# ekzhu/datasketch

Hardware: AMD Instinct MI355X
Metric: MinHash signatures/sec (1M sets x 256 tokens, num_perm=128) (higher is better)
Workload: dtype u64

## Files before the change

### datasketch_amd/csrc/mhx_api.hip

```cpp
#include <algorithm>
#include <cmath>
#include <condition_variable>
#include <cstdlib>
#include <cstring>
#include <mutex>
#include <new>
#include <system_error>
#include <thread>
#include <vector>

#include "mhx_internal.h"

namespace mhx {

static thread_local std::string g_last_error;

void set_error(const char *fmt, ...) {
    char buf[1024];
    va_list ap;
    va_start(ap, fmt);
    vsnprintf(buf, sizeof(buf), fmt, ap);
    va_end(ap);
    g_last_error = buf;
}
// ... 263 lines not shown

int mhx_ctx::ensure_copy_streams() {
    if (!copy_in) MHX_HIP_CHECK(hipStreamCreateWithFlags(&copy_in, hipStreamNonBlocking));
    if (!copy_out) MHX_HIP_CHECK(hipStreamCreateWithFlags(&copy_out, hipStreamNonBlocking));
    return MHX_OK;
}

int mhx_ctx::ensure_redo(int64_t n_sets) {
    if (n_sets <= redo_capacity && d_redo) return MHX_OK;
    if (d_redo) {
        (void)hipStreamSynchronize(stream);
        (void)mhx::dev_free(d_redo);
        d_redo = nullptr;
        redo_capacity = 0;
    }
    const int64_t cap = std::max<int64_t>(n_sets + n_sets / 4, 1024);
    hipError_t e = mhx::dev_malloc(reinterpret_cast<void **>(&d_redo), (size_t)cap + 64);
    if (e != hipSuccess) {
        d_redo = nullptr;
        return fail(MHX_ERR_OOM, "redo flag allocation of %lld bytes failed: %s", (long long)cap, hipGetErrorString(e));
    }
    redo_capacity = cap;
    return MHX_OK;
}

int mhx_ctx::ensure_work() {
    if (d_work) return MHX_OK;
    hipError_t e = mhx::dev_malloc(reinterpret_cast<void **>(&d_work), mhx::kWorkBytes);
    if (e != hipSuccess) {
        d_work = nullptr;
        return fail(MHX_ERR_OOM, "work counter allocation failed: %s", hipGetErrorString(e));
    }
    MHX_HIP_CHECK(hipMemsetAsync(d_work, 0, mhx::kWorkBytes, stream));
    return MHX_OK;
}

extern "C" {

const char *mhx_last_error(void) { return mhx::g_last_error.c_str(); }

const char *mhx_version(void) { return "mhx 0.1.0 (gfx950)"; }

int mhx_device_count(int *count) {
    if (!count) return fail(MHX_ERR_INVALID, "count is NULL");
    int n = 0;
    hipError_t e = hipGetDeviceCount(&n);
    if (e != hipSuccess) {
        (void)hipGetLastError();
        *count = 0;
        return MHX_OK;
    }
    *count = n;
    return MHX_OK;
}

int mhx_ctx_create(int device, mhx_ctx **out) {
    if (!out) return fail(MHX_ERR_INVALID, "ctx out pointer is NULL");
    *out = nullptr;
    int n = 0;
    if (hipGetDeviceCount(&n) != hipSuccess || n <= 0) {
        (void)hipGetLastError();
        return fail(MHX_ERR_NO_DEVICE, "no HIP device is available");
    }
    if (device < 0 || device >= n) return fail(MHX_ERR_INVALID, "device %d out of range [0,%d)", device, n);
    MHX_HIP_CHECK(hipSetDevice(device));
    hipDeviceProp_t prop;
    MHX_HIP_CHECK(hipGetDeviceProperties(&prop, device));
    mhx_ctx *ctx = new mhx_ctx();
    ctx->device = device;
    ctx->num_cus = prop.multiProcessorCount;
    ctx->lds_per_block = (int64_t)prop.sharedMemPerBlock;
    ctx->hbm_bytes = (int64_t)prop.totalGlobalMem;
    snprintf(ctx->name, sizeof(ctx->name), "%s (%s)", prop.name, prop.gcnArchName);
    hipError_t e = hipStreamCreateWithFlags(&ctx->stream, hipStreamNonBlocking);
    if (e != hipSuccess) {
        delete ctx;
        return fail(MHX_ERR_HIP, "hipStreamCreate failed: %s", hipGetErrorString(e));
    }
    *out = ctx;
    return MHX_OK;
}

int mhx_ctx_destroy(mhx_ctx *ctx) {
    if (!ctx) return MHX_OK;
    (void)hipSetDevice(ctx->device);
    (void)hipStreamSynchronize(ctx->stream);
    for (int i = 0; i < 5; ++i)
        if (ctx->scratch[i]) (void)mhx::dev_free(ctx->scratch[i]);
    if (ctx->d_stats) (void)mhx::dev_free(ctx->d_stats);
    if (ctx->d_redo) (void)mhx::dev_free(ctx->d_redo);
    if (ctx->d_work) (void)mhx::dev_free(ctx->d_work);
    if (ctx->copy_in) (void)hipStreamDestroy(ctx->copy_in);
    if (ctx->copy_out) (void)hipStreamDestroy(ctx->copy_out);
    (void)hipStreamDestroy(ctx->stream);
    delete ctx;
    return MHX_OK;
}

int mhx_ctx_synchronize(mhx_ctx *ctx) {
    MHX_ENTER(ctx, ctx);
    MHX_HIP_CHECK(hipStreamSynchronize(ctx->stream));
    return MHX_OK;
}

int mhx_ctx_release_scratch(mhx_ctx *ctx) {
    MHX_ENTER(ctx, ctx);
    MHX_TRY(ctx->activate());
    MHX_HIP_CHECK(hipStreamSynchronize(ctx->stream));
    for (int i = 0; i < 5; ++i) {
        if (ctx->scratch[i]) MHX_HIP_CHECK(mhx::dev_free(ctx->scratch[i]));
        ctx->scratch[i] = nullptr;
        ctx->scratch_bytes[i] = 0;
    }
    if (ctx->d_redo) {
        MHX_HIP_CHECK(mhx::dev_free(ctx->d_redo));
        ctx->d_redo = nullptr;
        ctx->redo_capacity = 0;
    }
    return MHX_OK;
}

int mhx_ctx_device_info(mhx_ctx *ctx, char *name, int name_len, int *cus, int64_t *hbm_bytes) {
    MHX_ENTER(ctx, ctx);
    if (name && name_len > 0) {
        strncpy(name, ctx->name, (size_t)name_len - 1);
        name[name_len - 1] = 0;
    }
    if (cus) *cus = ctx->num_cus;
    if (hbm_bytes) *hbm_bytes = ctx->hbm_bytes;
    return MHX_OK;
}

int mhx_ctx_set_option(mhx_ctx *ctx, const char *key, int64_t value) {
    static const struct {
        const char *key;
        int64_t mhx_ctx::*field;
    } options[] = {
        {"minhash.path", &mhx_ctx::opt_minhash_path},       {"minhash.split", &mhx_ctx::opt_minhash_split},
        {"minhash.packed", &mhx_ctx::opt_minhash_packed},   {"minhash.ties", &mhx_ctx::opt_minhash_ties},
        {"minhash.p3", &mhx_ctx::opt_minhash_p3},           {"minhash.share", &mhx_ctx::opt_minhash_share},
        {"minhash.adapt", &mhx_ctx::opt_minhash_adapt},     {"blocks_per_cu", &mhx_ctx::opt_blocks_per_cu},
        {"minhash.alias", &mhx_ctx::opt_minhash_alias},     {"minhash.prefetch", &mhx_ctx::opt_minhash_prefetch},
        {"weighted.path", &mhx_ctx::opt_weighted_path},     {"weighted.direct", &mhx_ctx::opt_weighted_direct},
        {"weighted.split", &mhx_ctx::opt_weighted_split},   {"weighted.tail", &mhx_ctx::opt_weighted_tail},
        {"weighted.debug", &mhx_ctx::opt_weighted_debug},   {"weighted.kernel", &mhx_ctx::opt_weighted_kernel},
        {"weighted.plan", &mhx_ctx::opt_weighted_plan},     {"weighted.rescue", &mhx_ctx::opt_weighted_rescue},
        {"weighted.min_dim", &mhx_ctx::opt_weighted_min_dim}, {"host.chunk_bytes", &mhx_ctx::opt_host_chunk_bytes},
        {"lsh.sort_bits", &mhx_ctx::opt_lsh_sort_bits},     {"lsh.gather", &mhx_ctx::opt_lsh_gather},
        {"lsh.sort", &mhx_ctx::opt_lsh_sort},               {"lsh.levels", &mhx_ctx::opt_lsh_levels},
        {"lsh.chunk", &mhx_ctx::opt_lsh_chunk},             {"lsh.team", &mhx_ctx::opt_lsh_team},
        {"lsh.bigbins", &mhx_ctx::opt_lsh_bigbins},         {"pack.fused", &mhx_ctx::opt_pack_fused},
        {"weighted.refill", &mhx_ctx::opt_weighted_refill}, {"lsh.prehash", &mhx_ctx::opt_lsh_prehash},
        {"lsh.merge_items", &mhx_ctx::opt_lsh_merge_items},
    };
    if (!ctx || !key) return fail(MHX_ERR_INVALID, "ctx/key is NULL");
    MHX_GUARD(ctx);
    for (const auto &o : options) {
        if (strcmp(key, o.key)) continue;
        if (o.field == &mhx_ctx::opt_lsh_merge_items)
            MHX_REQUIRE(value == 0 || value == 8 || value == 16, "lsh.merge_items must be 0, 8 or 16");
        ctx->*o.field = value;
        return MHX_OK;
    }
    return fail(MHX_ERR_INVALID, "unknown option '%s'", key);
}

int mhx_ctx_minhash_mode(mhx_ctx *ctx, int reset, int *mode) {
    MHX_ENTER(ctx, ctx);
    MHX_TRY(ctx->activate());
    MHX_TRY(ctx->ensure_work());
    unsigned int word = 0;
    MHX_HIP_CHECK(hipMemcpyAsync(&word, ctx->d_work + 8, sizeof(word), hipMemcpyDeviceToHost, ctx->stream));
    MHX_HIP_CHECK(hipStreamSynchronize(ctx->stream));
    if (mode) *mode = (int)word;
    if (reset) MHX_HIP_CHECK(hipMemsetAsync(ctx->d_work + 8, 0, sizeof(word), ctx->stream));
    return MHX_OK;
}

int mhx_ctx_minhash_flags(mhx_ctx *ctx, int64_t n_sets, uint8_t *flags) {
    MHX_ENTER(ctx, ctx);
    MHX_TRY(ctx->activate());
    MHX_REQUIRE(n_sets >= 0 && (flags || n_sets == 0), "NULL flags");
    if (ctx->redo_sets != n_sets || (n_sets > 0 && !ctx->d_redo))
        return fail(MHX_ERR_INVALID, "the last MinHash call on this context kept flags for %lld sets, not %lld (one huge set split over waves and "
                    "minhash.path != 0 keep none)", (long long)ctx->redo_sets, (long long)n_sets);
    MHX_HIP_CHECK(hipStreamSynchronize(ctx->stream));
    if (n_sets > 0) MHX_HIP_CHECK(hipMemcpy(flags, ctx->d_redo, (size_t)n_sets, hipMemcpyDeviceToHost));
    return MHX_OK;
}

int mhx_ctx_counters(mhx_ctx *ctx, int enable, uint64_t out[MHX_NUM_COUNTERS]) {
    MHX_ENTER(ctx, ctx);
    MHX_TRY(ctx->activate());
    MHX_HIP_CHECK(hipStreamSynchronize(ctx->stream));
    if (out) {
        for (int i = 0; i < MHX_NUM_COUNTERS; ++i) out[i] = 0;
        if (ctx->d_stats)
            MHX_HIP_CHECK(hipMemcpy(out, ctx->d_stats, sizeof(uint64_t) * MHX_NUM_COUNTERS, hipMemcpyDeviceToHost));
    }
    if (enable && !ctx->d_stats) {
        hipError_t e = mhx::dev_malloc(reinterpret_cast<void **>(&ctx->d_stats), sizeof(uint64_t) * MHX_NUM_COUNTERS);
        if (e != hipSuccess) {
            ctx->d_stats = nullptr;
            return fail(MHX_ERR_OOM, "counter allocation failed: %s", hipGetErrorString(e));
        }
    }
    if (!enable && ctx->d_stats) {
        MHX_HIP_CHECK(mhx::dev_free(ctx->d_stats));
// ... 1422 lines not shown
```

### datasketch_amd/csrc/mhx_internal.h

```cpp
#pragma once

#include <hip/hip_runtime.h>

#include <algorithm>
#include <cstdarg>
#include <cstdint>
#include <cstdio>
#include <mutex>
#include <string>
#include <unordered_map>

#include "mhx.h"

namespace mhx {

void set_error(const char *fmt, ...);
int fail(int code, const char *fmt, ...);
void forgive();

#define MHX_HIP_CHECK(expr)                                                                      \
    do {                                                                                         \
        hipError_t _e = (expr);                                                                  \
        if (_e != hipSuccess) {                                                                  \
            return ::mhx::fail(_e == hipErrorOutOfMemory ? MHX_ERR_OOM : MHX_ERR_HIP,            \
                               "%s failed: %s (%s:%d)", #expr, hipGetErrorString(_e), __FILE__,  \
                               __LINE__);                                                        \
        }                                                                                        \
    } while (0)

constexpr int kSigDigests = 2;
constexpr int kSigDigestsBM = 3;

constexpr unsigned int kPairListCap = 16384;
constexpr size_t kWorkBytes = 64 + sizeof(unsigned int) * kPairListCap;

#define MHX_GUARD(ctxp) std::lock_guard<std::recursive_mutex> _mhx_guard((ctxp)->mu)

#define MHX_REQUIRE(cond, ...)                                       \
    do {                                                             \
        if (!(cond)) return ::mhx::fail(MHX_ERR_INVALID, __VA_ARGS__); \
    } while (0)

hipError_t dev_malloc(void **p, size_t bytes, bool caller = false);
hipError_t dev_free(void *p);
bool guard_mode();

}

struct mhx_ctx {
    std::recursive_mutex mu;
    int device = 0;
    hipStream_t stream = nullptr;
    int num_cus = 0;
    int64_t lds_per_block = 64 << 10;
    int64_t hbm_bytes = 0;
    char name[128] = {0};
    void *scratch[5] = {nullptr, nullptr, nullptr, nullptr, nullptr};
    size_t scratch_bytes[5] = {0, 0, 0, 0, 0};
    int64_t opt_minhash_path = 0;
    int64_t opt_minhash_packed = 0;
    int64_t opt_minhash_adapt = 0;
    int64_t opt_minhash_share = 0;
    int64_t opt_minhash_p3 = 0;
    int64_t opt_minhash_ties = 0;
    int64_t opt_minhash_split = 0;
    int64_t opt_blocks_per_cu = 0;
    int64_t opt_minhash_prefetch = 1;
    int64_t opt_minhash_alias = -1;
    int64_t opt_weighted_path = 0;
    int64_t opt_weighted_min_dim = 0;
    int64_t opt_weighted_rescue = 0;
    int64_t opt_weighted_plan = 0;
    int64_t opt_weighted_kernel = 0;
    int64_t opt_weighted_debug = 0;
    int64_t opt_weighted_split = 0;
    int64_t opt_weighted_tail = 0;
    int64_t opt_weighted_direct = 0;
    int64_t opt_lsh_sort = 0;
    int64_t opt_lsh_gather = 0;
    int64_t opt_lsh_sort_bits = 0;
    int64_t opt_lsh_prehash = 0;
    int64_t opt_lsh_chunk = 0;
    int64_t opt_lsh_bigbins = 0;
    int64_t opt_lsh_team = 0;
    int64_t opt_lsh_merge_items = 0;
    int64_t opt_lsh_levels = 0;
    int64_t opt_pack_fused = 0;
    int64_t opt_weighted_refill = 0;
    int64_t opt_host_chunk_bytes = 0;

    hipStream_t copy_in = nullptr;
    hipStream_t copy_out = nullptr;
    int ensure_copy_streams();

    unsigned long long *d_stats = nullptr;
    uint8_t *d_redo = nullptr;
    int64_t redo_capacity = 0;
    int64_t redo_sets = 0;
    int ensure_redo(int64_t n_sets);
    unsigned int *d_work = nullptr;
    int ensure_work();

    int ensure_scratch(int slot, size_t bytes);
    int activate() const;
};

struct mhx_perm {
    mhx_ctx *ctx = nullptr;
    int32_t num_perm = 0;
    uint64_t *d_a = nullptr;
    uint64_t *d_b = nullptr;
};

struct mhx_wgen {
    mhx_ctx *ctx = nullptr;
    int32_t sample_size = 0;
    int32_t dim = 0;
    float *d_params = nullptr;
    int32_t s_pad = 0;
    bool table_fast = false;
    float *d_aos = nullptr;
    float *d_walk_a = nullptr;
    uint32_t *d_walk_c = nullptr;
    void *d_walk_plan = nullptr;
    int plan_index = 0;
    bool walk_ok = false;
};

struct mhx_event {
    mhx_ctx *ctx = nullptr;
    hipEvent_t ev = nullptr;
};

namespace mhx {
// ... 74 lines not shown
```

### datasketch_amd/csrc/minhash_kernels.hip

```cpp
#include <type_traits>

#include "mhx_internal.h"

namespace mhx {
namespace {

constexpr uint64_t kMersenne = (1ull << 61) - 1;
constexpr uint32_t kMaxHash = 0xFFFFFFFFu;
constexpr int kWave = 64;

struct BulkArgs {
    const void *hv;
    const int64_t *offsets;
    int64_t fixed_len;
    int64_t n_sets;
    const uint64_t *a;
    const uint64_t *b;
    int32_t num_perm;
    int32_t path;
    unsigned long long *stats;
    uint8_t *redo;
    int32_t redo_match;
    unsigned int *sieve_hint;
    unsigned int *mode_word;
    unsigned int *pair_count;
    unsigned int *pair_list;
    int32_t prefetch;
    int32_t ties;
    int32_t share_last;
    int64_t alias_mask;
    const uint64_t *init;
    int64_t init_stride;
    void *out;
};

__device__ __forceinline__ void mad_narrow(uint32_t h, uint32_t a_lo, uint32_t a_hi, uint64_t b,
                                           uint32_t &s_lo, uint32_t &s_hi) {
    const uint64_t s0 = (uint64_t)h * a_lo + b;
    s_lo = (uint32_t)s0;
    s_hi = (uint32_t)(s0 >> 32) + h * a_hi;
}

__device__ __forceinline__ void mad_wide(uint32_t h_lo, uint32_t h_hi, uint32_t a_lo, uint32_t a_hi,
                                         uint64_t b, uint32_t &s_lo, uint32_t &s_hi) {
    const uint64_t s0 = (uint64_t)h_lo * a_lo + b;
    s_lo = (uint32_t)s0;
    s_hi = (uint32_t)(s0 >> 32) + h_lo * a_hi + h_hi * a_lo;
}

__device__ __forceinline__ uint32_t fold_exact(uint32_t s_lo, uint32_t s_hi) {
    const uint32_t top = s_hi >> 29;
    const uint64_t y = ((((uint64_t)(s_hi & 0x1FFFFFFFu)) << 32) | s_lo) + top;
    return (uint32_t)y + (y >= kMersenne ? 1u : 0u);
}

__device__ __forceinline__ uint32_t fold_fast(uint32_t s_lo, uint32_t s_hi) {
    return s_lo + (s_hi >> 29);
}

// ... 672 lines not shown
#pragma unroll
        for (int p = 0; p < P; ++p) res[p] = m.v[p];
    }
}

template <int P, bool SHARE = false>
__device__ __forceinline__ void load_perms(const BulkArgs &args, int kbase, int lane, Perms<P> &pm,
                                           Perms<P> &pm_biased, SievePerms<P> &sp, int (&kidx)[P]) {
    uint32_t span = kWave;
    if constexpr (SHARE && P >= 3) {
        const int r = args.num_perm - (kbase + (P - 1) * kWave);
        span = r > 16 ? 32u : r > 8 ? 16u : r > 4 ? 8u : 4u;
    }
    sp.span = span;
#pragma unroll
    for (int p = 0; p < P; ++p) {
        const bool shared = SHARE && P >= 3 && p == P - 1;
        const int k = kbase + p * kWave + (shared ? lane & (int)(span - 1) : lane);
        const bool holds = k < args.num_perm;
        kidx[p] = holds && !(shared && lane >= (int)span) ? k : -1;
        const uint64_t a = holds ? args.a[k] : 0;
        pm.a_lo[p] = (uint32_t)a;
        pm.a_hi[p] = (uint32_t)(a >> 32);
        pm.b[p] = holds ? args.b[k] : 0;
        pm_biased.a_lo[p] = pm.a_lo[p];
        pm_biased.a_hi[p] = pm.a_hi[p];
        pm_biased.b[p] = pm.b[p] + 1;
        sp.a_lo[p] = pm.a_lo[p];
        sp.b8[p] = pm.b[p] + 8;
        sp.active[p] = kidx[p] >= 0;
    }
}

enum { MODE_SIEVE = 0, MODE_FULL = 1, MODE_DEDUP = 2, MODE_SIEVE_TIES = 3 };
enum { SHAPE_GENERAL = 0, SHAPE_PLAIN = 1, SHAPE_PLAIN_FIXED = 2, SHAPE_PLAIN_FIXED_ROWS = 3 };

template <int P, typename TokT, typename OutT, int MODE, int SHAPE, bool SHARE = false>
__global__ __launch_bounds__(256) void minhash_bulk_kernel(const BulkArgs args_in) {
    BulkArgs args = args_in;
    constexpr bool kSieve = MODE == MODE_SIEVE || MODE == MODE_SIEVE_TIES;
    if (kSieve && args.mode_word) {
        const unsigned int want_ties = *as_const(args.mode_word);
        if ((want_ties == 1u) != (MODE == MODE_SIEVE_TIES)) return;
    }
    if (MODE == MODE_FULL && args.mode_word && args.sieve_hint && blockIdx.x == 0 && threadIdx.x == 0) {
        const unsigned int t = __builtin_nontemporal_load(args.sieve_hint), f = __builtin_nontemporal_load(args.sieve_hint + 1);
        const unsigned int g = __builtin_nontemporal_load(args.sieve_hint + 2), m = *args.mode_word;
        const unsigned int tt = __builtin_nontemporal_load(args.sieve_hint + 3), tf = __builtin_nontemporal_load(args.sieve_hint + 5);
        if (t >= 64u) {
            const bool defeated = 4u * f > t;
            const bool heavy = m == 1u ? 5u * g > t : (tt >= 64u ? 5u * tf > tt : m == 2u);
            *args.mode_word = !defeated ? 0u : heavy ? 2u : 1u;
        }
    }
    if (SHAPE != SHAPE_GENERAL) {
        args.init = nullptr;
        args.init_stride = 0;
        args.stats = nullptr;
        args.alias_mask = -1;
    }
    if (SHAPE == SHAPE_PLAIN_FIXED || SHAPE == SHAPE_PLAIN_FIXED_ROWS) args.offsets = nullptr;
    const int lane = threadIdx.x & (kWave - 1);
    const int wave = __builtin_amdgcn_readfirstlane(threadIdx.x >> 6);
    const int waves_per_block = blockDim.x >> 6;
    const int kchunks = (args.num_perm + kWave * P - 1) / (kWave * P);
    constexpr int kLdsPerWave = MODE == MODE_DEDUP ? kDedupWordsPerWave : kStageWordsPerWave;
    __shared__ __attribute__((aligned(16))) uint32_t stage[4 * kLdsPerWave];
    uint32_t *lds = stage + wave * kLdsPerWave;
    Perms<P> pm, pm_biased;
    SievePerms<P> sp;
    int kidx[P];
    if (kSieve || MODE == MODE_DEDUP) load_perms<P, SHARE>(args, 0, lane, pm, pm_biased, sp, kidx);

    const TokT MHX_CONST_AS *hv = as_const(static_cast<const TokT *>(args.hv));
    const TokT *hv_vec = static_cast<const TokT *>(args.hv);
    const int64_t MHX_CONST_AS *offsets = as_const(args.offsets);
    OutT *__restrict__ out = static_cast<OutT *>(args.out);
    const int64_t stride = (int64_t)gridDim.x * waves_per_block;
    const bool flagged_only = !kSieve && args.redo != nullptr;
    unsigned int listed_n = 0;
    bool listed = false;
    if (MODE == MODE_FULL && flagged_only && args.pair_list) {
        listed_n = *as_const(args.pair_count);
        listed = listed_n <= kPairListCap;
    }
    const int64_t n_items = listed ? (int64_t)listed_n : flagged_only ? (args.n_sets + kWave - 1) / kWave * waves_per_block : args.n_sets;
    SieveBackoff backoff;
    TiesBackoff ties;
    int tried = 0, failed = 0, left = 0;
    if (MODE == MODE_SIEVE && args.sieve_hint) {
        const unsigned int t = __builtin_nontemporal_load(args.sieve_hint), f = __builtin_nontemporal_load(args.sieve_hint + 1);
        if (t >= 64u && 2u * f > t) {
            backoff.skip = 63;
            backoff.gap = 64;
            backoff.streak = 2;
        }
    }
    if (MODE == MODE_FULL && listed) {
        uint32_t *comb = stage;
        for (int64_t it = blockIdx.x; it < (int64_t)listed_n; it += gridDim.x) {
            const int64_t set = (int64_t)as_const(args.pair_list)[it];
            const int64_t beg = args.offsets ? offsets[set] : set * args.fixed_len;
            const int64_t end = args.offsets ? offsets[set + 1] : beg + args.fixed_len;
            const int64_t share = (end - beg + 31) / 32 * 8;
            const int64_t wbeg = min(end, beg + wave * share), wend = min(end, wbeg + share);
            for (int kc = 0; kc < kchunks; ++kc) {
                uint32_t mine[P];
#pragma unroll
                for (int p = 0; p < P; ++p) mine[p] = kMaxHash;
                if (wend > wbeg) {
                    const Minima<P> m = full_minima<P, TokT>(hv_vec, wbeg, wend, args.a, args.b, args.num_perm, kc * (kWave * P),
                                                             args.path == 1, args.stats);
#pragma unroll
                    for (int p = 0; p < P; ++p) mine[p] = m.v[p];
                }
#pragma unroll
                for (int p = 0; p < P; ++p) comb[(wave * P + p) * kWave + lane] = mine[p];
                __syncthreads();
                if (wave == 0) {
#pragma unroll
                    for (int p = 0; p < P; ++p) {
                        const int k = kc * (kWave * P) + p * kWave + lane;
                        if (k >= args.num_perm) continue;
                        uint32_t r = mine[p];
#pragma unroll
                        for (int w = 1; w < 4; ++w) r = min(r, comb[(w * P + p) * kWave + lane]);
                        uint64_t v = r;
                        if (args.init) {
                            const uint64_t iv = args.init[set * args.init_stride + k];
                            v = end > beg ? (uint64_t)min((iv >> 32) ? kMaxHash : (uint32_t)iv, r) : iv;
// ... 14 lines not shown
          const int64_t cand = item * kWave + lane;
          const bool mine = (lane % waves_per_block) == (int)(item0 % waves_per_block);
          todo = __ballot(mine && cand < args.n_sets && args.redo[cand] == (uint8_t)args.redo_match);
      }
      while (todo) {
        const int bit = __builtin_ctzll(todo);
        todo &= todo - 1;
        const int64_t set = listed ? (int64_t)as_const(args.pair_list)[item0] : flagged_only ? item * kWave + bit : item;
        int64_t beg, end;
        if (args.offsets) {
            beg = offsets[set];
            end = offsets[set + 1];
        } else {
            beg = (args.alias_mask >= 0 ? (set & args.alias_mask) : set) * args.fixed_len;
            end = beg + args.fixed_len;
        }
        uint32_t warm = 0;
        {
            const int64_t nset = listed ? args.n_sets : flagged_only ? (todo ? item * kWave + __builtin_ctzll(todo) : args.n_sets) : item + stride;
            const bool skipping_on = MODE == MODE_SIEVE && backoff.skip > 1;
            if (args.prefetch && nset < args.n_sets && !skipping_on) {
                const int64_t nbeg = args.offsets ? offsets[nset] : nset * args.fixed_len;
                const int64_t nend = args.offsets ? offsets[nset + 1] : nbeg + args.fixed_len;
                const int64_t off = (int64_t)lane * 128;
                if (off < (nend - nbeg) * (int64_t)sizeof(TokT))
                    warm = *reinterpret_cast<const volatile uint32_t *>(reinterpret_cast<const char *>(args.hv) +
                                                                         nbeg * (int64_t)sizeof(TokT) + off);
            }
        }
        bool defer = false;
        if (MODE == MODE_SIEVE && end > beg && backoff.skip > 0) {
            --backoff.skip;
            defer = true;
        }
        for (int kc = 0; kc < kchunks && !defer; ++kc) {
            uint32_t res[P];
            if (kSieve) {
                if (kchunks > 1) load_perms<P, SHARE>(args, kc * (kWave * P), lane, pm, pm_biased, sp, kidx);
                if (end > beg) {
                    bool tied = false;
                    defer = sieve_minima<P, TokT, SHAPE != SHAPE_PLAIN_FIXED_ROWS, MODE == MODE_SIEVE_TIES, SHARE>(hv, hv_vec, beg, end, pm, pm_biased, sp, args.stats, lane, lds, res,
                                                                                                          MODE == MODE_SIEVE_TIES ? &tied : nullptr);
                    if (kc == 0) ++tried;
                    if (MODE == MODE_SIEVE_TIES) {
                        if (defer || __any(tied)) ++failed;
                        if (defer) {
                            ++left;
                            break;
                        }
                    } else {
                        if (defer) {
                            ++failed;
                            backoff.failed();
                            break;
                        }
                        backoff.succeeded();
                    }
                }
            } else {
#pragma unroll
                for (int p = 0; p < P; ++p) {
                    const int k = kc * (kWave * P) + p * kWave + lane;
                    kidx[p] = k < args.num_perm ? k : -1;
                }
                if (end > beg) {
                    if (MODE == MODE_DEDUP) {
                        if (kchunks > 1) load_perms<P>(args, kc * (kWave * P), lane, pm, pm_biased, sp, kidx);
                        bool open = true;
                        if (!args.ties || (args.mode_word && *as_const(args.mode_word) == 1u)) {
                        } else if (ties.skip > 0) {
                            if (kc == kchunks - 1) --ties.skip;
                        } else {
                            open = sieve_minima<P, TokT, true, true>(hv, hv_vec, beg, end, pm, pm_biased, sp, nullptr, lane, lds, res);
                            if (kc == 0) ++tried, failed += open ? 1 : 0;
                            if (open) ties.failed(); else ties.succeeded();
                        }
                        if (open) {
#pragma unroll
                        for (int p = 0; p < P; ++p) res[p] = kMaxHash;
                        uint64_t cur[4];
                        load_quad<TokT>(hv_vec, beg, end, lane, cur);
                        defer = __any(dedup_sieve_range<P, TokT>(hv_vec, beg, end, pm, sp, lds, lane, cur, res));
                        if (defer) {
                            if (args.stats && lane == 0) atomicAdd(args.stats + 3, 1ull);
                            break;
                        }
// ... 18 lines not shown
                    } else {
                        v = iv;
                    }
                } else {
                    v = end > beg ? res[p] : kMaxHash;
                }
                if (sizeof(OutT) == 4) v = v > kMaxHash ? kMaxHash : v;
                out[set * args.num_perm + kidx[p]] = (OutT)v;
            }
        }
        if (kSieve && lane == 0) {
            args.redo[set] = defer ? 1 : 0;
            if (defer && args.stats) atomicAdd(args.stats, 1ull);
        }
        if (MODE == MODE_DEDUP && defer && lane == 0) {
            args.redo[set] = 2;
            if (args.pair_list) {
                const unsigned int slot = atomicAdd(args.pair_count, 1u);
                if (slot < kPairListCap) args.pair_list[slot] = (unsigned int)set;
            }
        }
        asm volatile("" ::"v"(warm));
      }
    }
    if (kSieve && args.sieve_hint && lane == 0 && wave == 0 && (blockIdx.x & 15u) == 0 && tried > 0) {
        atomicAdd(args.sieve_hint, (unsigned int)tried);
        if (failed) atomicAdd(args.sieve_hint + 1, (unsigned int)failed);
        if (left) atomicAdd(args.sieve_hint + 2, (unsigned int)left);
    }
    if (MODE == MODE_DEDUP && args.sieve_hint && args.mode_word && lane == 0 && tried > 0) {
        atomicAdd(args.sieve_hint + 3, (unsigned int)tried);
        if (failed) atomicAdd(args.sieve_hint + 5, (unsigned int)failed);
    }
}

template <int KP, int P, typename TokT, typename OutT>
__global__ __launch_bounds__(256) void minhash_packed_kernel(const BulkArgs args) {
    constexpr int G = kWave / KP;
    constexpr int STRIDE = 36;
    const int lane = threadIdx.x & (kWave - 1);
    const int wave = __builtin_amdgcn_readfirstlane(threadIdx.x >> 6);
    const int g = lane / KP, k = lane % KP;
    __shared__ __attribute__((aligned(16))) uint32_t stage[4 * G * kStageWordsPerWave];
    uint32_t *tiles = stage + wave * (G * kStageWordsPerWave);
    uint32_t *my_tile = tiles + g * kStageWordsPerWave;
    Perms<P> pm;
    SievePerms<P> sp;
    bool any_active = false;
#pragma unroll
    for (int q = 0; q < P; ++q) {
        const bool active = k + q * KP < args.num_perm;
        const uint64_t a = active ? args.a[k + q * KP] : 0, b = active ? args.b[k + q * KP] : 0;
        pm.a_lo[q] = sp.a_lo[q] = (uint32_t)a;
        pm.a_hi[q] = (uint32_t)(a >> 32);
        pm.b[q] = b;
        sp.b8[q] = b + 8;
        sp.active[q] = active;
        any_active |= active;
    }
    const TokT *hv_vec = static_cast<const TokT *>(args.hv);
    OutT *__restrict__ out = static_cast<OutT *>(args.out);
    const unsigned long long group_lanes = (KP == 64 ? ~0ull : ((1ull << KP) - 1ull)) << (g * KP);
    const int64_t n_items = (args.n_sets + G - 1) / G;
    for (int64_t item = (int64_t)blockIdx.x * 4 + wave; item < n_items; item += (int64_t)gridDim.x * 4) {
        const int64_t set = item * G + g;
        const bool has = set < args.n_sets;
// ... 190 lines not shown
#pragma unroll
        for (int u = 0; u < 4; ++u) {
            if (i + u * stride >= n2) break;
            ulonglong2 r;
            r.x = xa[u].x < ya[u].x ? xa[u].x : ya[u].x;
            r.y = xa[u].y < ya[u].y ? xa[u].y : ya[u].y;
            __builtin_nontemporal_store(r.x, &o2[i + u * stride].x);
            __builtin_nontemporal_store(r.y, &o2[i + u * stride].y);
        }
    }
    if ((count & 1) && blockIdx.x == 0 && threadIdx.x == 0)
        out[count - 1] = x[count - 1] < y[count - 1] ? x[count - 1] : y[count - 1];
}

unsigned resident_grid(mhx_ctx *ctx, const void *kernel, int64_t items) {
    int per_cu = 0;
    if (hipOccupancyMaxActiveBlocksPerMultiprocessor(&per_cu, kernel, 256, 0) != hipSuccess || per_cu < 1) {
        (void)hipGetLastError();
        per_cu = 2;
    }
    return (unsigned)std::max<int64_t>(1, std::min<int64_t>(items, (int64_t)ctx->num_cus * per_cu));
}

template <int P, typename TokT, typename OutT, int PF = P>
int launch_typed(mhx_ctx *ctx, const BulkArgs &args, int64_t first_token, int64_t total_tokens, bool split) {
    const int kchunks = (args.num_perm + kWave * P - 1) / (kWave * P);
    const int blocks_per_cu = ctx->opt_blocks_per_cu > 0 ? (int)ctx->opt_blocks_per_cu : (P >= 3 ? 128 : 64);
    const int64_t max_blocks = (int64_t)ctx->num_cus * blocks_per_cu;
    if (!split) {
        const int64_t want = (args.n_sets + 3) / 4;
        dim3 grid((unsigned)std::max<int64_t>(1, std::min(want, max_blocks)), 1u);
        if (args.path == 0) {
            if (int rc = ctx->ensure_work()) return rc;
            MHX_HIP_CHECK(hipMemsetAsync(ctx->d_work, 0, 8 * sizeof(unsigned int), ctx->stream));
            BulkArgs sieve_args = args;
            sieve_args.sieve_hint = ctx->d_work;
            sieve_args.mode_word = ctx->opt_minhash_adapt == 1 || args.stats ? nullptr : ctx->d_work + 8;
            const BulkArgs &args_s = sieve_args;
            const bool plain = !args.init && !args.stats && args.alias_mask < 0;
            const int np = args.num_perm;
            const bool packable = !args.stats && args.alias_mask < 0 && ctx->opt_minhash_packed != 1;
            const bool packed = packable && P <= 2 && (np <= 96 || (ctx->opt_minhash_packed == 2 && np <= 128));
            if (packed) {
                const int kp = np <= 8 ? 8 : np <= 16 ? 16 : np <= 32 ? 32 : np <= 64 ? 16 : np <= 96 ? 32 : 64;
                const int64_t items = (args.n_sets + 64 / kp - 1) / (64 / kp);
                dim3 pgrid((unsigned)std::max<int64_t>(1, std::min<int64_t>((items + 3) / 4, max_blocks)), 1u);
#define MHX_PACKED(KP_, P_) hipLaunchKernelGGL((minhash_packed_kernel<KP_, P_, TokT, OutT>), pgrid, dim3(256), 0, ctx->stream, args_s)
                if (np <= 8) MHX_PACKED(8, 1);
                else if (np <= 16) MHX_PACKED(16, 1);
                else if (np <= 32) MHX_PACKED(32, 1);
                else if (np <= 48) MHX_PACKED(16, 3);
                else if (np <= 64) MHX_PACKED(16, 4);
                else if (np <= 96) MHX_PACKED(32, 3);
                else MHX_PACKED(64, 2);
#undef MHX_PACKED
            } else {
            const bool fixed_rows = plain && !args.offsets && args.fixed_len % kRowTokens == 0;
            const int last_slot = args.num_perm - (P - 1) * kWave;
            const bool share = P >= 3 && kchunks == 1 && args.share_last && last_slot > 0 && last_slot <= 32;
            const auto first_launches = [&](auto share_tag) {
                constexpr bool SH = decltype(share_tag)::value;
#define MHX_SIEVE(MODE_, SHAPE_) hipLaunchKernelGGL((minhash_bulk_kernel<P, TokT, OutT, MODE_, SHAPE_, SH>), grid, dim3(256), 0, ctx->stream, args_s)
                if (fixed_rows) MHX_SIEVE(MODE_SIEVE, SHAPE_PLAIN_FIXED_ROWS);
                else if (plain && !args.offsets) MHX_SIEVE(MODE_SIEVE, SHAPE_PLAIN_FIXED);
                else if (plain) MHX_SIEVE(MODE_SIEVE, SHAPE_PLAIN);
                else MHX_SIEVE(MODE_SIEVE, SHAPE_GENERAL);
                if (args_s.mode_word) {
                    if (fixed_rows) MHX_SIEVE(MODE_SIEVE_TIES, SHAPE_PLAIN_FIXED_ROWS);
                    else MHX_SIEVE(MODE_SIEVE_TIES, SHAPE_GENERAL);
                }
#undef MHX_SIEVE
            };
            if constexpr (P >= 3) {
                if (share) first_launches(std::true_type());
                else first_launches(std::false_type());
            } else {
                (void)share;
                first_launches(std::false_type());
            }
            }
            const int64_t flag_groups = (args.n_sets + kWave - 1) / kWave;
            BulkArgs dedup = args;
            dedup.redo_match = 1;
            dedup.sieve_hint = sieve_args.sieve_hint;
            dedup.mode_word = packed ? nullptr : sieve_args.mode_word;
            if (args.n_sets <= 0xFFFFFFFFll) {
                dedup.pair_count = ctx->d_work + 4;
                dedup.pair_list = ctx->d_work + 16;
            }
            hipLaunchKernelGGL((minhash_bulk_kernel<PF, TokT, OutT, MODE_DEDUP, SHAPE_GENERAL>),
                               dim3(resident_grid(ctx, (const void *)minhash_bulk_kernel<PF, TokT, OutT, MODE_DEDUP, SHAPE_GENERAL>, flag_groups)),
                               dim3(256), 0, ctx->stream, dedup);
            BulkArgs rest = dedup;
            rest.redo_match = 2;
            hipLaunchKernelGGL((minhash_bulk_kernel<PF, TokT, OutT, MODE_FULL, SHAPE_GENERAL>),
                               dim3(resident_grid(ctx, (const void *)minhash_bulk_kernel<PF, TokT, OutT, MODE_FULL, SHAPE_GENERAL>, flag_groups)),
                               dim3(256), 0, ctx->stream, rest);
        } else {
            BulkArgs all = args;
            all.redo = nullptr;
            hipLaunchKernelGGL((minhash_bulk_kernel<PF, TokT, OutT, MODE_FULL, SHAPE_GENERAL>), grid, dim3(256), 0, ctx->stream, all);
        }
    } else {
        const int64_t total_out = args.n_sets * (int64_t)args.num_perm;
        const int64_t fill_blocks = std::max<int64_t>(1, std::min<int64_t>((total_out + 255) / 256, max_blocks));
        hipLaunchKernelGGL((minhash_fill_state_kernel<OutT>), dim3((unsigned)fill_blocks), dim3(256), 0,
                           ctx->stream, args);
        const int64_t waves = (int64_t)ctx->num_cus * 32;
        int64_t slice = (total_tokens + waves - 1) / waves;
        slice = slice > 128 ? (slice + 255) / 256 * 256 : std::max<int64_t>(64, (slice + 15) / 16 * 16);
        const int64_t n_slices = (total_tokens + slice - 1) / slice;
        const int64_t want = (n_slices + 3) / 4;
        dim3 grid((unsigned)std::max<int64_t>(1, std::min(want, max_blocks)), (unsigned)kchunks);
        hipLaunchKernelGGL((minhash_split_kernel<P, TokT, OutT>), grid, dim3(256), 0, ctx->stream, args,
                           first_token, total_tokens, slice);
    }
    MHX_HIP_CHECK(hipGetLastError());
    return MHX_OK;
}

template <typename TokT, typename OutT>
// ... 4 lines not shown
    int best = 2;
    if (may3 && slots(3) <= slots(best)) best = 3;
    if (may4 && slots(4) <= slots(best)) best = 4;
    if (best == 3) return launch_typed<3, TokT, OutT, 2>(ctx, args, first_token, total_tokens, split);
    if (best == 4) return launch_typed<4, TokT, OutT, 2>(ctx, args, first_token, total_tokens, split);
    return launch_typed<2, TokT, OutT>(ctx, args, first_token, total_tokens, split);
}

}

int launch_minhash_bulk(mhx_perm *perm, const void *d_hv, int hv_dtype, const int64_t *d_offsets,
                        int64_t fixed_len, int64_t n_sets, int64_t total_tokens,
                        const uint64_t *d_init, int64_t init_stride, void *d_out, int out_dtype, int64_t first_token) {
    mhx_ctx *ctx = perm->ctx;
    if (n_sets == 0) return MHX_OK;
    total_tokens -= first_token;
    BulkArgs args;
    args.hv = d_hv;
    args.offsets = d_offsets;
    args.fixed_len = fixed_len;
    args.n_sets = n_sets;
    args.a = perm->d_a;
    args.b = perm->d_b;
    args.num_perm = perm->num_perm;
    args.path = (int32_t)ctx->opt_minhash_path;
    args.stats = ctx->d_stats;
    args.redo = nullptr;
    args.redo_match = 1;
    args.sieve_hint = nullptr;
    args.mode_word = nullptr;
    args.alias_mask = ctx->opt_minhash_alias;
    args.pair_count = nullptr;
    args.pair_list = nullptr;
    args.prefetch = ctx->opt_minhash_prefetch == 2 || (ctx->opt_minhash_prefetch == 1 && (d_offsets != nullptr || fixed_len < 256));
    args.ties = ctx->opt_minhash_ties != 1;
    args.share_last = ctx->opt_minhash_share != 1;
    args.init = d_init;
    args.init_stride = init_stride;
    args.out = d_out;
    const int64_t waves_avail = (int64_t)ctx->num_cus * 16;
    bool split = n_sets < waves_avail && total_tokens > n_sets * 128 && total_tokens >= 1024;
    if (ctx->opt_minhash_split == 1) split = false;
    if (ctx->opt_minhash_split == 2) split = total_tokens > 0;
    ctx->redo_sets = 0;
    if (!split && args.path == 0) {
        if (int rc = ctx->ensure_redo(n_sets)) return rc;
        args.redo = ctx->d_redo;
        ctx->redo_sets = n_sets;
    }
    if (hv_dtype == MHX_U64 && out_dtype == MHX_U64) return launch_p<uint64_t, uint64_t>(ctx, args, first_token, total_tokens, split);
    if (hv_dtype == MHX_U64 && out_dtype == MHX_U32) return launch_p<uint64_t, uint32_t>(ctx, args, first_token, total_tokens, split);
    if (hv_dtype == MHX_U32 && out_dtype == MHX_U64) return launch_p<uint32_t, uint64_t>(ctx, args, first_token, total_tokens, split);
    if (hv_dtype == MHX_U32 && out_dtype == MHX_U32) return launch_p<uint32_t, uint32_t>(ctx, args, first_token, total_tokens, split);
    return fail(MHX_ERR_INVALID, "unknown hv_dtype/out_dtype (%d, %d)", hv_dtype, out_dtype);
}

int launch_minhash_merge(mhx_ctx *ctx, const uint64_t *d_x, const uint64_t *d_y, int64_t count,
                         uint64_t *d_out) {
    if (count == 0) return MHX_OK;
    const int64_t want = ((count >> 1) + 1023) / 1024;
    const int64_t blocks = std::max<int64_t>(1, std::min<int64_t>(want, (int64_t)ctx->num_cus * 32));
    hipLaunchKernelGGL(minhash_merge_kernel, dim3((unsigned)blocks), dim3(256), 0, ctx->stream, d_x, d_y,
                       count, d_out);
    MHX_HIP_CHECK(hipGetLastError());
    return MHX_OK;
}
// ... 3 lines not shown
```

Baseline: 499.8 million.

## Replace dedup+full follow-up passes with a single list-driven settle kernel

Sieve kernels now append deferred or failed sets to sharded per-context lists in the work buffer. When the previous call reported, through a mapped host summary word, that the lists did not overflow, the host skips the redundant sieve/ties launch and the dedup and full passes, and launches one settle kernel. That kernel reprocesses only the listed sets and resets the counters itself with a last-block ticket. This removes a memset and one or two extra kernel launches plus full redo-flag scans, at the cost of host-side state that depends on the previous call and extra atomics in the sieve kernels.

```diff
diff --git a/datasketch_amd/csrc/mhx_api.hip b/datasketch_amd/csrc/mhx_api.hip
--- a/datasketch_amd/csrc/mhx_api.hip
+++ b/datasketch_amd/csrc/mhx_api.hip
@@ -319,6 +319,16 @@
         return fail(MHX_ERR_OOM, "work counter allocation failed: %s", hipGetErrorString(e));
     }
     MHX_HIP_CHECK(hipMemsetAsync(d_work, 0, mhx::kWorkBytes, stream));
+    if (hipHostMalloc(reinterpret_cast<void **>(&h_summary), 64, hipHostMallocMapped) == hipSuccess) {
+        *h_summary = 0;
+        if (hipHostGetDevicePointer(reinterpret_cast<void **>(&d_summary), h_summary, 0) != hipSuccess) {
+            (void)hipHostFree(h_summary);
+            h_summary = d_summary = nullptr;
+        }
+    } else {
+        h_summary = nullptr;
+    }
+    if (!h_summary) (void)hipGetLastError();
     return MHX_OK;
 }
 
@@ -377,6 +387,7 @@
     if (ctx->d_stats) (void)mhx::dev_free(ctx->d_stats);
     if (ctx->d_redo) (void)mhx::dev_free(ctx->d_redo);
     if (ctx->d_work) (void)mhx::dev_free(ctx->d_work);
+    if (ctx->h_summary) (void)hipHostFree(ctx->h_summary);
     if (ctx->copy_in) (void)hipStreamDestroy(ctx->copy_in);
     if (ctx->copy_out) (void)hipStreamDestroy(ctx->copy_out);
     (void)hipStreamDestroy(ctx->stream);
@@ -427,6 +438,7 @@
         {"minhash.packed", &mhx_ctx::opt_minhash_packed},   {"minhash.ties", &mhx_ctx::opt_minhash_ties},
         {"minhash.p3", &mhx_ctx::opt_minhash_p3},           {"minhash.share", &mhx_ctx::opt_minhash_share},
         {"minhash.adapt", &mhx_ctx::opt_minhash_adapt},     {"blocks_per_cu", &mhx_ctx::opt_blocks_per_cu},
+        {"minhash.settle", &mhx_ctx::opt_minhash_settle},   {"minhash.listcap", &mhx_ctx::opt_minhash_listcap},
         {"minhash.alias", &mhx_ctx::opt_minhash_alias},     {"minhash.prefetch", &mhx_ctx::opt_minhash_prefetch},
         {"weighted.path", &mhx_ctx::opt_weighted_path},     {"weighted.direct", &mhx_ctx::opt_weighted_direct},
         {"weighted.split", &mhx_ctx::opt_weighted_split},   {"weighted.tail", &mhx_ctx::opt_weighted_tail},
@@ -446,6 +458,8 @@
         if (strcmp(key, o.key)) continue;
         if (o.field == &mhx_ctx::opt_lsh_merge_items)
             MHX_REQUIRE(value == 0 || value == 8 || value == 16, "lsh.merge_items must be 0, 8 or 16");
+        if (o.field == &mhx_ctx::opt_minhash_listcap)
+            MHX_REQUIRE(value >= 0 && value <= (int64_t)mhx::kSettleListCap, "minhash.listcap must be in [0, %u]", mhx::kSettleListCap);
         ctx->*o.field = value;
         return MHX_OK;
     }
@@ -460,7 +474,10 @@
     MHX_HIP_CHECK(hipMemcpyAsync(&word, ctx->d_work + 8, sizeof(word), hipMemcpyDeviceToHost, ctx->stream));
     MHX_HIP_CHECK(hipStreamSynchronize(ctx->stream));
     if (mode) *mode = (int)word;
-    if (reset) MHX_HIP_CHECK(hipMemsetAsync(ctx->d_work + 8, 0, sizeof(word), ctx->stream));
+    if (reset) {
+        MHX_HIP_CHECK(hipMemsetAsync(ctx->d_work + 8, 0, sizeof(word), ctx->stream));
+        if (ctx->h_summary) *ctx->h_summary &= ~mhx::kSummaryModeMask;
+    }
     return MHX_OK;
 }
 
diff --git a/datasketch_amd/csrc/mhx_internal.h b/datasketch_amd/csrc/mhx_internal.h
--- a/datasketch_amd/csrc/mhx_internal.h
+++ b/datasketch_amd/csrc/mhx_internal.h
@@ -32,7 +32,14 @@
 constexpr int kSigDigestsBM = 3;
 
 constexpr unsigned int kPairListCap = 16384;
-constexpr size_t kWorkBytes = 64 + sizeof(unsigned int) * kPairListCap;
+constexpr unsigned int kSettleShards = 16;
+constexpr unsigned int kSettleListCap = 256;
+constexpr unsigned int kWorkShardCount = 16;
+constexpr unsigned int kWorkTicket = 32;
+constexpr unsigned int kWorkShardList = 64;
+constexpr unsigned int kWorkPairList = kWorkShardList + kSettleShards * kSettleListCap;
+constexpr size_t kWorkBytes = sizeof(unsigned int) * (kWorkPairList + kPairListCap);
+constexpr unsigned int kSummaryValid = 0x100u, kSummaryComplete = 0x10u, kSummaryModeMask = 0xFu;
 
 #define MHX_GUARD(ctxp) std::lock_guard<std::recursive_mutex> _mhx_guard((ctxp)->mu)
 
@@ -60,6 +67,8 @@
     int64_t opt_minhash_path = 0;
     int64_t opt_minhash_packed = 0;
     int64_t opt_minhash_adapt = 0;
+    int64_t opt_minhash_settle = 1;
+    int64_t opt_minhash_listcap = 0;
     int64_t opt_minhash_share = 0;
     int64_t opt_minhash_p3 = 0;
     int64_t opt_minhash_ties = 0;
@@ -100,6 +109,8 @@
     int ensure_redo(int64_t n_sets);
     unsigned int *d_work = nullptr;
     int ensure_work();
+    unsigned int *h_summary = nullptr;
+    unsigned int *d_summary = nullptr;
 
     int ensure_scratch(int slot, size_t bytes);
     int activate() const;
diff --git a/datasketch_amd/csrc/minhash_kernels.hip b/datasketch_amd/csrc/minhash_kernels.hip
--- a/datasketch_amd/csrc/minhash_kernels.hip
+++ b/datasketch_amd/csrc/minhash_kernels.hip
@@ -25,6 +25,10 @@
     unsigned int *mode_word;
     unsigned int *pair_count;
     unsigned int *pair_list;
+    unsigned int *work;
+    unsigned int *summary;
+    int32_t list_cap;
+    int32_t first_forced;
     int32_t prefetch;
     int32_t ties;
     int32_t share_last;
@@ -763,6 +767,16 @@
     }
 }
 
+__device__ __forceinline__ unsigned int next_mode(const unsigned int *hint, unsigned int m) {
+    const auto word = [&](int i) { return __hip_atomic_load(hint + i, __ATOMIC_RELAXED, __HIP_MEMORY_SCOPE_AGENT); };
+    const unsigned int t = word(0), f = word(1), g = word(2);
+    const unsigned int tt = word(3), tf = word(5);
+    if (t < 64u) return m;
+    const bool defeated = 4u * f > t;
+    const bool heavy = m == 1u ? 5u * g > t : (tt >= 64u ? 5u * tf > tt : m == 2u);
+    return !defeated ? 0u : heavy ? 2u : 1u;
+}
+
 enum { MODE_SIEVE = 0, MODE_FULL = 1, MODE_DEDUP = 2, MODE_SIEVE_TIES = 3 };
 enum { SHAPE_GENERAL = 0, SHAPE_PLAIN = 1, SHAPE_PLAIN_FIXED = 2, SHAPE_PLAIN_FIXED_ROWS = 3 };
 
@@ -770,18 +784,25 @@
 __global__ __launch_bounds__(256) void minhash_bulk_kernel(const BulkArgs args_in) {
     BulkArgs args = args_in;
     constexpr bool kSieve = MODE == MODE_SIEVE || MODE == MODE_SIEVE_TIES;
-    if (kSieve && args.mode_word) {
+    if (kSieve && args.mode_word && !args.first_forced) {
         const unsigned int want_ties = *as_const(args.mode_word);
         if ((want_ties == 1u) != (MODE == MODE_SIEVE_TIES)) return;
     }
-    if (MODE == MODE_FULL && args.mode_word && args.sieve_hint && blockIdx.x == 0 && threadIdx.x == 0) {
-        const unsigned int t = __builtin_nontemporal_load(args.sieve_hint), f = __builtin_nontemporal_load(args.sieve_hint + 1);
-        const unsigned int g = __builtin_nontemporal_load(args.sieve_hint + 2), m = *args.mode_word;
-        const unsigned int tt = __builtin_nontemporal_load(args.sieve_hint + 3), tf = __builtin_nontemporal_load(args.sieve_hint + 5);
-        if (t >= 64u) {
-            const bool defeated = 4u * f > t;
-            const bool heavy = m == 1u ? 5u * g > t : (tt >= 64u ? 5u * tf > tt : m == 2u);
-            *args.mode_word = !defeated ? 0u : heavy ? 2u : 1u;
+    if (MODE == MODE_FULL && args.sieve_hint && blockIdx.x == 0 && threadIdx.x == 0) {
+        unsigned int mode = 0u;
+        if (args.mode_word) {
+            mode = next_mode(args.sieve_hint, *args.mode_word);
+            *args.mode_word = mode;
+        }
+        for (int i = 0; i < 8; ++i)
+            if (i != 4) args.sieve_hint[i] = 0u;
+        if (args.work) {
+            bool complete = true;
+            for (unsigned int s = 0; s < kSettleShards; ++s) {
+                complete = complete && __hip_atomic_load(args.work + kWorkShardCount + s, __ATOMIC_RELAXED, __HIP_MEMORY_SCOPE_AGENT) <= (unsigned int)args.list_cap;
+                args.work[kWorkShardCount + s] = 0u;
+            }
+            if (args.summary) __hip_atomic_store(args.summary, kSummaryValid | (complete ? kSummaryComplete : 0u) | mode, __ATOMIC_RELAXED, __HIP_MEMORY_SCOPE_SYSTEM);
         }
     }
     if (SHAPE != SHAPE_GENERAL) {
@@ -818,6 +839,7 @@
     const int64_t n_items = listed ? (int64_t)listed_n : flagged_only ? (args.n_sets + kWave - 1) / kWave * waves_per_block : args.n_sets;
     SieveBackoff backoff;
     TiesBackoff ties;
+    bool list_open = kSieve && args.work != nullptr;
     int tried = 0, failed = 0, left = 0;
     if (MODE == MODE_SIEVE && args.sieve_hint) {
         const unsigned int t = __builtin_nontemporal_load(args.sieve_hint), f = __builtin_nontemporal_load(args.sieve_hint + 1);
@@ -826,7 +848,21 @@
             backoff.gap = 64;
             backoff.streak = 2;
         }
-    }
+        if (f > kSettleShards * (unsigned int)args.list_cap) list_open = false;
+    }
+    if (MODE == MODE_SIEVE_TIES && args.sieve_hint && list_open &&
+        __builtin_nontemporal_load(args.sieve_hint + 2) > kSettleShards * (unsigned int)args.list_cap)
+        list_open = false;
+    const auto list_append = [&](int64_t set) {
+        if (!list_open) return;
+        unsigned int slot = 0;
+        if (lane == 0) {
+            const unsigned int shard = blockIdx.x & (kSettleShards - 1);
+            slot = atomicAdd(args.work + kWorkShardCount + shard, 1u);
+            if (slot < (unsigned int)args.list_cap) args.work[kWorkShardList + shard * kSettleListCap + slot] = (unsigned int)set;
+        }
+        if ((unsigned int)__builtin_amdgcn_readfirstlane((int)slot) >= (unsigned int)args.list_cap) list_open = false;
+    };
     if (MODE == MODE_FULL && listed) {
         uint32_t *comb = stage;
         for (int64_t it = blockIdx.x; it < (int64_t)listed_n; it += gridDim.x) {
@@ -907,6 +943,7 @@
         if (MODE == MODE_SIEVE && end > beg && backoff.skip > 0) {
             --backoff.skip;
             defer = true;
+            list_append(set);
         }
         for (int kc = 0; kc < kchunks && !defer; ++kc) {
             uint32_t res[P];
@@ -921,12 +958,14 @@
                         if (defer || __any(tied)) ++failed;
                         if (defer) {
                             ++left;
+                            list_append(set);
                             break;
                         }
                     } else {
                         if (defer) {
                             ++failed;
                             backoff.failed();
+                            list_append(set);
                             break;
                         }
                         backoff.succeeded();
@@ -1011,6 +1050,187 @@
         atomicAdd(args.sieve_hint + 3, (unsigned int)tried);
         if (failed) atomicAdd(args.sieve_hint + 5, (unsigned int)failed);
     }
+}
+
+template <int P, typename TokT, typename OutT>
+__global__ __launch_bounds__(256) void minhash_settle_kernel(const BulkArgs args) {
+    const int lane = threadIdx.x & (kWave - 1);
+    const int wave = __builtin_amdgcn_readfirstlane(threadIdx.x >> 6);
+    const int kchunks = (args.num_perm + kWave * P - 1) / (kWave * P);
+    __shared__ __attribute__((aligned(16))) uint32_t stage[4 * kDedupWordsPerWave];
+    __shared__ long long pend[4];
+    uint32_t *lds = stage + wave * kDedupWordsPerWave;
+    Perms<P> pm, pm_biased;
+    SievePerms<P> sp;
+    int kidx[P];
+    load_perms<P>(args, 0, lane, pm, pm_biased, sp, kidx);
+    const TokT MHX_CONST_AS *hv = as_const(static_cast<const TokT *>(args.hv));
+    const TokT *hv_vec = static_cast<const TokT *>(args.hv);
+    const int64_t MHX_CONST_AS *offsets = as_const(args.offsets);
+    OutT *__restrict__ out = static_cast<OutT *>(args.out);
+    const unsigned int cap = (unsigned int)args.list_cap;
+    const bool ties_done = args.first_forced == 2 || !args.ties;
+    TiesBackoff ties;
+    int tried = 0, failed = 0;
+
+    const auto settle = [&](int64_t set) {
+        bool open = false;
+        int64_t beg = 0, end = 0;
+        if (set >= 0) {
+            beg = args.offsets ? offsets[set] : set * args.fixed_len;
+            end = args.offsets ? offsets[set + 1] : beg + args.fixed_len;
+            {
+                const int64_t off = (int64_t)lane * 128;
+                uint32_t warm = 0;
+                if (off < (end - beg) * (int64_t)sizeof(TokT))
+                    warm = *reinterpret_cast<const volatile uint32_t *>(reinterpret_cast<const char *>(args.hv) + beg * (int64_t)sizeof(TokT) + off);
+                asm volatile("" ::"v"(warm));
+            }
+            for (int kc = 0; kc < kchunks && !open; ++kc) {
+                uint32_t res[P];
+                if (kchunks > 1) load_perms<P>(args, kc * (kWave * P), lane, pm, pm_biased, sp, kidx);
+                if (end > beg) {
+                    bool dedup = true;
+                    if (ties_done) {
+                    } else if (ties.skip > 0) {
+                        if (kc == kchunks - 1) --ties.skip;
+                    } else {
+                        dedup = sieve_minima<P, TokT, true, true>(hv, hv_vec, beg, end, pm, pm_biased, sp, nullptr, lane, lds, res);
+                        if (kc == 0) ++tried, failed += dedup ? 1 : 0;
+                        if (dedup) ties.failed(); else ties.succeeded();
+                    }
+                    if (dedup) {
+#pragma unroll
+                        for (int p = 0; p < P; ++p) res[p] = kMaxHash;
+                        uint64_t cur[4];
+                        load_quad<TokT>(hv_vec, beg, end, lane, cur);
+                        open = __any(dedup_sieve_range<P, TokT>(hv_vec, beg, end, pm, sp, lds, lane, cur, res));
+                        if (open) break;
+                    }
+                }
+#pragma unroll
+                for (int p = 0; p < P; ++p) {
+                    if (kidx[p] < 0) continue;
+                    uint64_t v = end > beg ? res[p] : kMaxHash;
+                    out[set * args.num_perm + kidx[p]] = (OutT)v;
+                }
+            }
+            if (open && lane == 0) args.redo[set] = 2;
+        }
+        if (lane == 0) pend[wave] = open ? (long long)set : -1ll;
+        __syncthreads();
+        uint32_t *comb = stage;
+        for (int w = 0; w < 4; ++w) {
+            const int64_t pset = (int64_t)pend[w];
+            if (pset < 0) continue;
+            const int64_t pbeg = args.offsets ? offsets[pset] : pset * args.fixed_len;
+            const int64_t pend_tok = args.offsets ? offsets[pset + 1] : pbeg + args.fixed_len;
+            const int64_t share = (pend_tok - pbeg + 31) / 32 * 8;
+            const int64_t wbeg = min(pend_tok, pbeg + wave * share), wend = min(pend_tok, wbeg + share);
+            for (int kc = 0; kc < kchunks; ++kc) {
+                uint32_t mine[P];
+#pragma unroll
+                for (int p = 0; p < P; ++p) mine[p] = kMaxHash;
+                if (wend > wbeg) {
+                    const Minima<P> m = full_minima<P, TokT>(hv_vec, wbeg, wend, args.a, args.b, args.num_perm, kc * (kWave * P), false, nullptr);
+#pragma unroll
+                    for (int p = 0; p < P; ++p) mine[p] = m.v[p];
+                }
+#pragma unroll
+                for (int p = 0; p < P; ++p) comb[(wave * P + p) * kWave + lane] = mine[p];
+                __syncthreads();
+                if (wave == 0) {
+#pragma unroll
+                    for (int p = 0; p < P; ++p) {
+                        const int k = kc * (kWave * P) + p * kWave + lane;
+                        if (k >= args.num_perm) continue;
+                        uint32_t r = mine[p];
+#pragma unroll
+                        for (int q = 1; q < 4; ++q) r = min(r, comb[(q * P + p) * kWave + lane]);
+                        out[pset * args.num_perm + k] = (OutT)(uint64_t)r;
+                    }
+                }
+                __syncthreads();
+            }
+        }
+        __syncthreads();
+    };
+
+    unsigned int total = 0;
+    bool complete = true;
+    for (unsigned int s = 0; s < kSettleShards; ++s) {
+        const unsigned int c = as_const(args.work)[kWorkShardCount + s];
+        complete = complete && c <= cap;
+        total += c;
+    }
+    if (complete) {
+        for (int64_t base = (int64_t)blockIdx.x * 4; base < (int64_t)total; base += (int64_t)gridDim.x * 4) {
+            int64_t set = -1;
+            unsigned int i = (unsigned int)base + (unsigned int)wave;
+            if (i < total) {
+                unsigned int s = 0;
+                for (; s < kSettleShards - 1; ++s) {
+                    const unsigned int c = as_const(args.work)[kWorkShardCount + s];
+                    if (i < c) break;
+                    i -= c;
+                }
+                set = (int64_t)as_const(args.work)[kWorkShardList + s * kSettleListCap + i];
+            }
+            settle(set);
+        }
+    } else {
+        const int64_t chunks = (args.n_sets + 1023) / 1024;
+        for (int64_t chunk = blockIdx.x; chunk < chunks; chunk += gridDim.x) {
+            const int64_t first = chunk * 1024 + 16 * lane;
+            uint32_t mask = 0;
+            if (first + 16 <= args.n_sets) {
+                const uint4 q = *reinterpret_cast<const uint4 *>(args.redo + first);
+                const uint32_t w4[4] = {q.x, q.y, q.z, q.w};
+#pragma unroll
+                for (int j = 0; j < 16; ++j) mask |= ((w4[j >> 2] >> (8 * (j & 3))) & 255u) == 1u ? 1u << j : 0u;
+            } else {
+                for (int j = 0; j < 16; ++j)
+                    if (first + j < args.n_sets && args.redo[first + j] == 1) mask |= 1u << j;
+            }
+            unsigned long long lanes = __ballot(mask != 0u);
+            uint32_t bits = 0;
+            int from = 0;
+            while (lanes || bits) {
+                int64_t set = -1;
+                for (int w = 0; w < 4; ++w) {
+                    if (!bits) {
+                        if (!lanes) break;
+                        from = __builtin_ctzll(lanes);
+                        lanes &= lanes - 1;
+                        bits = (uint32_t)__builtin_amdgcn_readlane((int)mask, from);
+                    }
+                    const int b = __builtin_ctz(bits);
+                    bits &= bits - 1;
+                    if (w == wave) set = chunk * 1024 + 16 * from + b;
+                }
+                settle(set);
+            }
+        }
+    }
+    if (lane == 0 && tried > 0 && args.sieve_hint && args.mode_word) {
+        atomicAdd(args.sieve_hint + 3, (unsigned int)tried);
+        if (failed) atomicAdd(args.sieve_hint + 5, (unsigned int)failed);
+    }
+    __syncthreads();
+    if (threadIdx.x != 0) return;
+    __threadfence();
+    if (atomicAdd(args.work + kWorkTicket, 1u) != gridDim.x - 1) return;
+    __threadfence();
+    unsigned int mode = 0u;
+    if (args.mode_word) {
+        const unsigned int was = *args.mode_word, ran = args.first_forced == 2 ? 1u : was == 1u ? 0u : was;
+        mode = args.sieve_hint ? next_mode(args.sieve_hint, ran) : was;
+        *args.mode_word = mode;
+    }
+    for (int i = 0; i < 8; ++i) args.work[i] = 0u;
+    for (unsigned int s = 0; s < kSettleShards; ++s) args.work[kWorkShardCount + s] = 0u;
+    args.work[kWorkTicket] = 0u;
+    if (args.summary) __hip_atomic_store(args.summary, kSummaryValid | (complete ? kSummaryComplete : 0u) | mode, __ATOMIC_RELAXED, __HIP_MEMORY_SCOPE_SYSTEM);
 }
 
 template <int KP, int P, typename TokT, typename OutT>
@@ -1267,15 +1487,24 @@
         dim3 grid((unsigned)std::max<int64_t>(1, std::min(want, max_blocks)), 1u);
         if (args.path == 0) {
             if (int rc = ctx->ensure_work()) return rc;
-            MHX_HIP_CHECK(hipMemsetAsync(ctx->d_work, 0, 8 * sizeof(unsigned int), ctx->stream));
-            BulkArgs sieve_args = args;
-            sieve_args.sieve_hint = ctx->d_work;
-            sieve_args.mode_word = ctx->opt_minhash_adapt == 1 || args.stats ? nullptr : ctx->d_work + 8;
-            const BulkArgs &args_s = sieve_args;
             const bool plain = !args.init && !args.stats && args.alias_mask < 0;
             const int np = args.num_perm;
             const bool packable = !args.stats && args.alias_mask < 0 && ctx->opt_minhash_packed != 1;
             const bool packed = packable && P <= 2 && (np <= 96 || (ctx->opt_minhash_packed == 2 && np <= 128));
+            const bool lists = plain && !packed && ctx->opt_minhash_settle != 0 && ctx->d_summary && args.n_sets <= 0xFFFFFFFFll;
+            const unsigned int summary = lists ? *static_cast<volatile unsigned int *>(ctx->h_summary) : 0u;
+            const bool settle = (summary & kSummaryValid) && (summary & kSummaryComplete);
+            if (!settle) MHX_HIP_CHECK(hipMemsetAsync(ctx->d_work, 0, 8 * sizeof(unsigned int), ctx->stream));
+            BulkArgs sieve_args = args;
+            if (lists) {
+                sieve_args.work = ctx->d_work;
+                sieve_args.summary = ctx->d_summary;
+                sieve_args.list_cap = (int32_t)(ctx->opt_minhash_listcap > 0 ? ctx->opt_minhash_listcap : (int64_t)kSettleListCap);
+            }
+            sieve_args.sieve_hint = ctx->d_work;
+            sieve_args.mode_word = ctx->opt_minhash_adapt == 1 || args.stats ? nullptr : ctx->d_work + 8;
+            if (settle) sieve_args.first_forced = sieve_args.mode_word && (summary & kSummaryModeMask) == 1u ? 2 : 1;
+            const BulkArgs &args_s = sieve_args;
             if (packed) {
                 const int kp = np <= 8 ? 8 : np <= 16 ? 16 : np <= 32 ? 32 : np <= 64 ? 16 : np <= 96 ? 32 : 64;
                 const int64_t items = (args.n_sets + 64 / kp - 1) / (64 / kp);
@@ -1296,11 +1525,12 @@
             const auto first_launches = [&](auto share_tag) {
                 constexpr bool SH = decltype(share_tag)::value;
 #define MHX_SIEVE(MODE_, SHAPE_) hipLaunchKernelGGL((minhash_bulk_kernel<P, TokT, OutT, MODE_, SHAPE_, SH>), grid, dim3(256), 0, ctx->stream, args_s)
-                if (fixed_rows) MHX_SIEVE(MODE_SIEVE, SHAPE_PLAIN_FIXED_ROWS);
+                if (args_s.first_forced == 2) {
+                } else if (fixed_rows) MHX_SIEVE(MODE_SIEVE, SHAPE_PLAIN_FIXED_ROWS);
                 else if (plain && !args.offsets) MHX_SIEVE(MODE_SIEVE, SHAPE_PLAIN_FIXED);
                 else if (plain) MHX_SIEVE(MODE_SIEVE, SHAPE_PLAIN);
                 else MHX_SIEVE(MODE_SIEVE, SHAPE_GENERAL);
-                if (args_s.mode_word) {
+                if (args_s.mode_word && args_s.first_forced != 1) {
                     if (fixed_rows) MHX_SIEVE(MODE_SIEVE_TIES, SHAPE_PLAIN_FIXED_ROWS);
                     else MHX_SIEVE(MODE_SIEVE_TIES, SHAPE_GENERAL);
                 }
@@ -1315,13 +1545,19 @@
             }
             }
             const int64_t flag_groups = (args.n_sets + kWave - 1) / kWave;
-            BulkArgs dedup = args;
+            if (settle) {
+                hipLaunchKernelGGL((minhash_settle_kernel<PF, TokT, OutT>),
+                                   dim3(resident_grid(ctx, (const void *)minhash_settle_kernel<PF, TokT, OutT>, std::max<int64_t>(std::min<int64_t>(kSettleShards * kSettleListCap / 4, (args.n_sets + 3) / 4), (args.n_sets + 1023) / 1024))),
+                                   dim3(256), 0, ctx->stream, sieve_args);
+                MHX_HIP_CHECK(hipGetLastError());
+                return MHX_OK;
+            }
+            BulkArgs dedup = sieve_args;
             dedup.redo_match = 1;
-            dedup.sieve_hint = sieve_args.sieve_hint;
             dedup.mode_word = packed ? nullptr : sieve_args.mode_word;
             if (args.n_sets <= 0xFFFFFFFFll) {
                 dedup.pair_count = ctx->d_work + 4;
-                dedup.pair_list = ctx->d_work + 16;
+                dedup.pair_list = ctx->d_work + kWorkPairList;
             }
             hipLaunchKernelGGL((minhash_bulk_kernel<PF, TokT, OutT, MODE_DEDUP, SHAPE_GENERAL>),
                                dim3(resident_grid(ctx, (const void *)minhash_bulk_kernel<PF, TokT, OutT, MODE_DEDUP, SHAPE_GENERAL>, flag_groups)),
@@ -1392,6 +1628,10 @@
     args.alias_mask = ctx->opt_minhash_alias;
     args.pair_count = nullptr;
     args.pair_list = nullptr;
+    args.work = nullptr;
+    args.summary = nullptr;
+    args.list_cap = 0;
+    args.first_forced = 0;
     args.prefetch = ctx->opt_minhash_prefetch == 2 || (ctx->opt_minhash_prefetch == 1 && (d_offsets != nullptr || fixed_len < 256));
     args.ties = ctx->opt_minhash_ties != 1;
     args.share_last = ctx->opt_minhash_share != 1;
```

New measurement: 502.7 million, median of 6. Within noise of the previous version (+0.6%).
